# Fytex/Shafa-CD

Measured on AMD Instinct MI355X. Metric: GiB/s Shannon-Fano encode+decode, 64 MiB blocks, 1/2/4/8 GPUs; bit-exact, higher is better.
Workload: dtype u8

## Files before the change

### shafa-cd_amd/csrc/api.hip

```cpp
#include "common.hpp"
#include "internal.hpp"

#include <cmath>
#include <stdio.h>
#include <stdlib.h>

#include <mutex>

static thread_local char g_last_error[512] = "";

int shafa_set_hip_error(hipError_t e, const char *what)
{
    snprintf(g_last_error, sizeof(g_last_error), "%s: %s", what, hipGetErrorString(e));
    return SHAFA_DEVICE_ERROR;
}

int batch_enter(Batch *b, hipStream_t st)
{
    if (!b) return SHAFA_OUTSIDE_MODULE;
    int dev = -1;
    HIP_TRY(hipGetDevice(&dev));
    if (dev != b->device) {
        snprintf(g_last_error, sizeof(g_last_error), "batch of device %d used while device %d is current", b->device, dev);
        return SHAFA_DEVICE_ERROR;
// ... 259 lines not shown

int shafa_hip_set_option(const char *name, long value)
{
    if (name && !strcmp(name, "sf_encode_one_pass_min_blocks")) {
        sfenc_configure(value < 0 ? 0 : (value > (1 << 30) ? (1 << 30) : (int)value));
        return SHAFA_SUCCESS;
    }
    if (name && !strcmp(name, "sf_encode_window_bits")) {
        extern int g_sfe_window_bits;
        if (value < 0 || value > 16) return SHAFA_OUTSIDE_MODULE;
        g_sfe_window_bits = (int)value;
        return SHAFA_SUCCESS;
    }
    if (name && !strcmp(name, "sf_encode_lanes")) {
        if (value != 0 && value != 256 && value != 512) return SHAFA_OUTSIDE_MODULE;
        g_sfe_lanes = (int)value;
        return SHAFA_SUCCESS;
    }
    if (name && !strcmp(name, "sf_decode_path")) {
        if (value < 0 || value > 2) return SHAFA_OUTSIDE_MODULE;
        sfdec_configure_path((int)value);
        return SHAFA_SUCCESS;
    }
    if (name && !strcmp(name, "rle_encode_general")) {
        rleenc_configure(value != 0);
        return SHAFA_SUCCESS;
    }
    if (name && !strcmp(name, "rle_encode_one_pass"))
        return value == 0 ? SHAFA_SUCCESS : SHAFA_OUTSIDE_MODULE;
    if (name && !strcmp(name, "sf_decode_speculate")) {
        sfdec_configure(value <= 0 ? 0 : value >= 2 ? 2 : 1);
        return SHAFA_SUCCESS;
    }
    return SHAFA_OUTSIDE_MODULE;
}

int shafa_hipd_batch_create(int max_blocks, size_t max_block_bytes, shafa_hipd_batch **out)
{
    if (!out || max_blocks <= 0) return SHAFA_OUTSIDE_MODULE;
    Batch *b = (Batch *)calloc(1, sizeof(Batch));
    if (!b) return SHAFA_LACK_OF_MEMORY;
    b->max_blocks = max_blocks;
    b->max_block_bytes = max_block_bytes;
    if (hipGetDevice(&b->device) != hipSuccess) { free(b); return SHAFA_DEVICE_ERROR; }
    b->h_hosterr = (int *)calloc((size_t)max_blocks, sizeof(int));
    if (!b->h_hosterr) { free(b); return SHAFA_LACK_OF_MEMORY; }
    hipError_t e = hipMalloc((void **)&b->d_err, (size_t)max_blocks * sizeof(int));
    if (e == hipSuccess) e = hipMemset(b->d_err, 0, (size_t)max_blocks * sizeof(int));
    if (e == hipSuccess) e = hipMalloc(&b->d_par_hist, (size_t)max_blocks * 48);
    if (e == hipSuccess) e = hipHostMalloc((void **)&b->h_err, (size_t)max_blocks * sizeof(int), hipHostMallocDefault);
    if (e != hipSuccess) {
        if (b->d_err) hipFree(b->d_err);
        free(b);
        return shafa_set_hip_error(e, "shafa_hipd_batch_create");
    }
    *out = (shafa_hipd_batch *)b;
    return SHAFA_SUCCESS;
}

void shafa_hipd_batch_destroy(shafa_hipd_batch *hb)
{
    Batch *b = (Batch *)hb;
    if (!b) return;
    DeviceGuard dg(b->device);
    if (b->has_last) (void)hipStreamSynchronize(b->last_st);
    hipDeviceSynchronize();
// ... 895 lines not shown
```

### shafa-cd_amd/csrc/internal.hpp

```cpp
#pragma once

#include "common.hpp"

#include <string.h>
#include <vector>

struct StageSeg {
    size_t off, bytes;
    hipStream_t st;
    hipEvent_t ev;
    bool sealed;
};

constexpr size_t PARAMS_INLINE_BYTES = 64 * 1024;

struct Batch {
    int device;
    hipStream_t last_st;
    bool has_last;
    int max_blocks;
    size_t max_block_bytes;
    void *d_ws;
    size_t ws_bytes;
    u8 *h_stage;
// ... 200 lines not shown
enum ErrSrc { ERR_PAIR = 0, ERR_QUANT = 1, ERR_ROUND = 2 };
struct ErrorArgs {
    ErrSrc src;
    const u32 *h_mant, *h_keep;
    const double *h_step, *h_bound, *h_abs, *h_rel;
    const u8 *d_ref;
    const u64 *h_ref_off;
};
int planes_error_launch_dev(Batch *bt, hipStream_t st, int nblocks, u32 elem, const ErrorArgs &e, const u8 *d_el, const u64 *h_off,
                            const u64 *h_cap, const u64 *d_n, u64 *d_stat);
int records_launch_dev(Batch *bt, hipStream_t st, int nblocks, u32 width, bool merge, u8 *d_rec, const u64 *h_off, const u64 *h_cap,
                       const u64 *d_n, u8 *d_planes, const u64 *h_plane_off);
int seek_index_launch_dev(Batch *bt, hipStream_t st, int nblocks, const u8 *d_in, const u64 *h_in_off, const u64 *h_in_cap,
                          const u64 *d_in_n, const shafa_code_table *d_tables, u32 span, int flags, const u64 *h_ckpt_first,
                          u64 *d_ckpt, u32 *d_status, u64 *d_out_n);
int read_spans_launch_dev(Batch *bt, hipStream_t st, int nblocks, const u8 *d_file, const u64 *h_pay_off, const u64 *h_pay_n,
                          const u64 *h_n_symbols, const u64 *h_ckpt_first, const shafa_code_table *d_tables, u32 span, int flags,
                          const u64 *d_ckpt, int nitems, const int *h_item_block, const u64 *h_item_first,
                          const u64 *h_item_last, const u64 *h_item_lo, const u64 *h_item_hi, const u64 *h_item_dst, u8 *d_out);
int sfesize_launch_dev(Batch *bt, hipStream_t st, int nblocks, const u64 *d_freq, const shafa_code_table *d_tables, u64 *d_out_n);
struct MoveDesc {
    const u8 *src;
    u8 *dst;
    u64 n;
    u64 hdr_val;
    u32 hdr_len;
    u32 pad;
};
int pack_move_launch(hipStream_t st, int nblocks, const MoveDesc *d_bulk, const MoveDesc *d_seam, const u32 *d_verdict,
                     u64 max_n);
void sfenc_configure(int sfe4_min_blocks);
void sfdec_configure(int speculate);
void sfdec_configure_path(int path);
void rleenc_configure(int force_general);
int gen_launch(hipStream_t st, u64 seed, u64 first, const u8 *d_map, u8 *d_out, size_t n);

int api_lazy_init();
int api_pipe_device(int slot, int n_slots);
```

### shafa-cd_amd/csrc/sf_decode.hip

```cpp
#include <type_traits>
#include "common.hpp"
#include "internal.hpp"

#include <atomic>
#include <mutex>
#include <thread>

#include <algorithm>

#include <stdlib.h>

#include "sfd_common.hpp"
#include "sfd_dp.hpp"
#include "sfd_generic.hpp"

namespace {

typedef __attribute__((address_space(3))) u32 lds_u32;
typedef __attribute__((address_space(3))) u16 lds_u16;
typedef __attribute__((address_space(3))) u8 lds_u8;
template <int LONG> constexpr u32 spec_emask() { return LONG == 2 ? 31u : 15u; }

constexpr int SC_PHW = 16;
constexpr int SC_M = 4;
constexpr int SC_SB = SC_PHW * 4 * SC_M;
constexpr int SC_CH = SC_SB / CH_BYTES;
constexpr int SC_STRIPS_TILE = DTILE / SC_SB;
constexpr int SC_WTILES = 64 / SC_STRIPS_TILE;
constexpr int SC_TILES = DEC_THREADS / SC_STRIPS_TILE;
constexpr int SC_ROWW = SC_PHW + 1;
constexpr int SC_COLB = DEC_THREADS * 4;
constexpr int SC_LDS_ROWS = SC_ROWW * SC_COLB;
constexpr int SC_MISC = 64;
static_assert(SC_COLB == 1024 && SC_WTILES == 2 && SC_STRIPS_TILE == 32, "sfd_scan's lane maps");

struct ScanWin {
    u32 lo, hi, wa, cb;
    __device__ __forceinline__ void init(u32 col) { cb = col; wa = 0xFFFFFFFFu; hi = lo = 0; }
    __device__ __forceinline__ void flush() { wa = 0xFFFFFFFFu; }
    __device__ __forceinline__ u32 at(u32 q)
    {
        const u32 a = cb + ((q >> 5) << 10);
        if (a != wa) {
            lo = *(const lds_u32 *)(size_t)a;
            hi = *(const lds_u32 *)(size_t)(a + SC_COLB);
            wa = a;
        }
        return __builtin_amdgcn_alignbit(hi, lo, q);
    }
};

template <int LONG>
__device__ __forceinline__ u32 scan_long_len(const u16 *lt, ScanWin &sw, const u32 qq)
{
    const u32 win = __builtin_bitreverse32(sw.at(qq));
    const u32 l = (LONG == 1 ? long_code(lt, win) : long_code32(lt, win)) >> 8;
    return l ? l : 1u;
}

template <int LONG>
__device__ __forceinline__ void scan_multi(const lds_u8 *tab, const u16 *lt, const u32 KW, u32 &q, const u32 qe, u32 &cnt, ScanWin &sw)
{
    const u32 q0 = q;
    u32 acc = 0;
    auto multi = [&](auto nlook) {
        constexpr u32 N = decltype(nlook)::value;
        const u32 in_row = 32u * SC_PHW - 1u - (LONG ? (N - 1u) * KW : 0u);
// ... 9 lines not shown
            acc += sum;
            q += sum & 31u;
            if (LONG && __builtin_expect((e & 31u) == 0u, 0)) {
                const u32 l = scan_long_len<LONG>(lt, sw, q);
                q += l;
                acc += l + 32u;
            }
        }
    };
    if (KW <= 10) multi(std::integral_constant<u32, 3>{});
    else multi(std::integral_constant<u32, 2>{});
    cnt += (acc - (q - q0)) >> 5;
}

template <bool LAST, int LONG>
__device__ __forceinline__ bool scan_single(const lds_u8 *tab, const u16 *lt, const u32 KW, u32 &q, const u32 qe, const int qlimit,
                                            u32 &cnt, ScanWin &sw)
{
    const u32 mask = (1u << KW) - 1u;
    const lds_u8 *len0 = tab + (1u << KW);
    while (q < qe) {
        u32 l0 = len0[sw.at(q) & mask];
        if (LONG && __builtin_expect(l0 == 0u, 0)) l0 = scan_long_len<LONG>(lt, sw, q);
        if (LAST && (int)(q + l0) > qlimit) return true;
        q += l0;
        ++cnt;
    }
    return false;
}

#define SC_QUAD 0
#define SC_WAVES 6
#define SC_NT 0
struct ScanIO {
    const u8 *in;
    u64 in_n;
    long long grp_off;
    u32 wbase, ph, cb;
    static constexpr u32 G = SC_QUAD ? 4u : 2u, SPL = 64u / G;
    __device__ __forceinline__ void init(const DecBlk &blk, const u64 wave_off)
    {
        const u32 tid = threadIdx.x, lane = tid & 63u, px = lane / G;
        in = blk.in;
        in_n = blk.in_n;
        ph = lane % G;
        grp_off = (long long)wave_off + (long long)px * SC_SB + 16ll * ph;
        wbase = 4u * ((tid & ~63u) + px);
        cb = 4u * tid;
    }
    template <bool CHECKED>
    __device__ __forceinline__ uint4 fetch16(const long long off) const
    {
        if (!CHECKED || (off >= 0 && (u64)off + 16 <= in_n)) return SC_NT ? gload_nt<uint4>(in + off) : gload<uint4>(in + off);
        u32 w0 = 0, w1 = 0, w2 = 0, w3 = 0;
        if (off >= 0 && (u64)off < in_n) {
            const int nv = (int)(in_n - (u64)off);
#pragma clang loop unroll(disable)
            for (int b = 0; b < nv; ++b) {
                const u32 v = (u32)gload<u8>(in + off + b) << (8 * (b & 3));
                const int wi = b >> 2;
                w0 |= wi == 0 ? v : 0u;
                w1 |= wi == 1 ? v : 0u;
                w2 |= wi == 2 ? v : 0u;
                w3 |= wi == 3 ? v : 0u;
            }
        }
        return make_uint4(w0, w1, w2, w3);
    }
    static __device__ __forceinline__ constexpr u32 sgrp(const int t) { return SC_QUAD ? (u32)t : (u32)t >> 1; }
    static __device__ __forceinline__ constexpr u32 piece(const int t) { return SC_QUAD ? 0u : 32u * ((u32)t & 1u); }
    template <bool CHECKED>
    __device__ __forceinline__ void load_phase(const int k, uint4 (&R)[4]) const
    {
#pragma unroll
        for (int t = 0; t < 4; ++t)
            R[t] = fetch16<CHECKED>(grp_off + (long long)sgrp(t) * SPL * SC_SB + 64ll * k + piece(t));
    }
    template <bool CHECKED>
    __device__ __forceinline__ void load_line(const int j, uint4 (&R)[8]) const
    {
#pragma unroll
        for (int g = 0; g < 2; ++g)
#pragma unroll
            for (int h = 0; h < 2; ++h)
#pragma unroll
                for (int u = 0; u < 2; ++u) {
                    const int t = 2 * g + u;
                    R[4 * h + t] = fetch16<CHECKED>(grp_off + (long long)sgrp(t) * SPL * SC_SB + 64ll * (2 * j + h) + piece(t));
                }
    }
    static constexpr int NRU = SC_QUAD ? 4 : 2;
    template <bool CHECKED>
    __device__ __forceinline__ void load_runup(uint4 (&RU)[NRU]) const
    {
#pragma unroll
        for (int t = 0; t < NRU; ++t) {
            const long long o = grp_off - 32ll - (SC_QUAD ? 16ll * (ph & 2u) : 0ll) + (long long)t * SPL * SC_SB;
            RU[t] = fetch16<CHECKED>(o < 0 ? o + 32 : o);
        }
    }
    __device__ __forceinline__ void put(const u32 r, const u32 xhi, const u32 v) const
    {
        *(lds_u32 *)(size_t)(wbase + r * SC_COLB + 4u * SPL * xhi) = rev_bytes(v);
    }
    __device__ __forceinline__ void wave_sync() const
    {
        __builtin_amdgcn_fence(__ATOMIC_ACQ_REL, "wavefront", "local");
        __builtin_amdgcn_wave_barrier();
    }
    __device__ __forceinline__ void put_runup(const uint4 (&RU)[NRU]) const
    {
#pragma unroll
        for (int t = 0; t < NRU; ++t) {
            const u32 r = 9u + 4u * (ph & 1u);
            if (!SC_QUAD || ph < 2u) {
                put(r, t, RU[t].x);
                put(r + 1, t, RU[t].y);
                put(r + 2, t, RU[t].z);
                put(r + 3, t, RU[t].w);
            }
        }
        wave_sync();
    }
    __device__ __forceinline__ void put_phase(const uint4 *R) const
    {
        const u32 carry = *(const lds_u32 *)(size_t)(cb + 16u * SC_COLB);
        wave_sync();
#pragma unroll
        for (int t = 0; t < 4; ++t) {
            const u32 r = 1u + 4u * ph + piece(t) / 4u;
            put(r, sgrp(t), R[t].x);
            put(r + 1, sgrp(t), R[t].y);
            put(r + 2, sgrp(t), R[t].z);
            put(r + 3, sgrp(t), R[t].w);
        }
        *(lds_u32 *)(size_t)cb = carry;
        wave_sync();
    }
    __device__ __forceinline__ u32 next_strip_word(const uint4 *R, const u64 wave_off) const
    {
        const u32 lane = threadIdx.x & 63u;
        if (ph == 0) {
            if (lane) *(lds_u32 *)(size_t)(wbase - 4u) = rev_bytes(R[0].x);
            *(lds_u32 *)(size_t)(wbase - 4u + 4u * SPL) = rev_bytes(R[2].x);
        }
        wave_sync();
        u32 nw = *(const lds_u32 *)(size_t)cb;
        if (lane == 63) nw = rev_bytes(gload<u32>(in + wave_off + (u64)64 * SC_SB));
        wave_sync();
        return nw;
    }
    __device__ __forceinline__ void put_next_word(const u32 nw_rev) const
    {
        const u32 carry = *(const lds_u32 *)(size_t)(cb + 16u * SC_COLB);
        *(lds_u32 *)(size_t)cb = carry;
        *(lds_u32 *)(size_t)(cb + SC_COLB) = nw_rev;
    }
    template <bool CHECKED>
    __device__ __forceinline__ void put_next_strip(const u64 wave_off) const
    {
        u32 nw = 0;
        const long long off = (long long)wave_off + (long long)((threadIdx.x & 63u) + 1u) * SC_SB;
        if (!CHECKED || (u64)off + 4 <= in_n) nw = gload<u32>(in + off);
        else {
#pragma unroll
            for (int b = 0; b < 4; ++b)
                if ((u64)off + b < in_n) nw |= (u32)gload<u8>(in + off + b) << (8 * b);
        }
        const u32 carry = *(const lds_u32 *)(size_t)(cb + 16u * SC_COLB);
        *(lds_u32 *)(size_t)cb = carry;
        *(lds_u32 *)(size_t)(cb + SC_COLB) = rev_bytes(nw);
    }
};

struct ScanOut {
    u32 e[2], c[4];
    __device__ __forceinline__ void clear() { e[0] = e[1] = 0; c[0] = c[1] = c[2] = c[3] = 0; }
    template <int J> __device__ __forceinline__ void put_ent(const u32 v) { e[J >> 2] |= v << (8 * (J & 3)); }
    template <int J> __device__ __forceinline__ void put_cnt(const u32 v) { c[J >> 1] |= v << (16 * (J & 1)); }
    __device__ __forceinline__ u32 ent(const u32 j) const { return ((j < 4 ? e[0] : e[1]) >> (8u * (j & 3u))) & 0xFFu; }
    __device__ __forceinline__ void set_ent(const u32 j, const u32 v)
    {
        const u32 sh = 8u * (j & 3u), m = ~(0xFFu << sh), x = v << sh;
        if (j < 4) e[0] = (e[0] & m) | x; else e[1] = (e[1] & m) | x;
    }
    __device__ __forceinline__ void set_cnt(const u32 j, const u32 v)
    {
        const u32 sh = 16u * (j & 1u), m = ~(0xFFFFu << sh), x = v << sh, i = j >> 1;
        c[0] = i == 0 ? (c[0] & m) | x : c[0];
        c[1] = i == 1 ? (c[1] & m) | x : c[1];
        c[2] = i == 2 ? (c[2] & m) | x : c[2];
        c[3] = i == 3 ? (c[3] & m) | x : c[3];
    }
    __device__ __forceinline__ u32 total() const
    {
        u32 t = 0;
#pragma unroll
        for (int i = 0; i < 4; ++i) t += (c[i] & 0xFFFFu) + (c[i] >> 16);
        return t;
    }
};
static_assert(SC_CH == 8, "ScanOut packs eight chunks");

template <int LONG>
__device__ __forceinline__ void scan_strip_fast(const lds_u8 *tab, const u16 *lt, const u32 KW, const DecBlk &blk, const u64 wave_off,
                                                const u32 e_forced, const bool forced, ScanOut &o, u32 &exit_)
{
    o.clear();
    ScanIO io;
    io.init(blk, wave_off);
    ScanWin sw;
    sw.init(io.cb);
#ifndef SC_LINE
#define SC_LINE 1
#endif
    uint4 R[SC_LINE ? 8 : 4];
    u32 q, pc = 0;
    auto to_row_end = [&]() {
        scan_multi<LONG>(tab, lt, KW, q, 32u * SC_PHW + 32u, pc, sw);
        if (LONG) scan_single<false, LONG>(tab, lt, KW, q, 32u * SC_PHW, 0, pc, sw);
    };
    {
        uint4 RU[ScanIO::NRU];
        io.load_runup<false>(RU);
#if SC_LINE
        io.load_line<false>(0, R);
#else
        io.load_phase<false>(0, R);
#endif
        io.put_runup(RU);
    }
    static_assert(!SC_QUAD, "next_strip_word: pair mapping");
    const u32 nextw = io.next_strip_word(R, wave_off);
    q = 32u * 9u;
    to_row_end();
    q -= 32u * SC_PHW;
    auto phase = [&](auto kc) {
        constexpr int k = decltype(kc)::value;
#if SC_LINE
        io.put_phase(R + 4 * (k & 1));
        sw.flush();
        if ((k & 1) && k + 1 < SC_M) io.load_line<false>((k + 1) / 2, R);
#else
        io.put_phase(R);
        sw.flush();
        if (k + 1 < SC_M) io.load_phase<false>(k + 1, R);
#endif
        scan_single<false, LONG>(tab, lt, KW, q, 32u, 0, pc, sw);
        if (k > 0) o.put_cnt<(k > 0 ? 2 * k - 1 : 0)>(pc);
        if (k == 0 && forced) q = 32u + e_forced;
        o.put_ent<2 * k>(q - 32u);
        u32 c = 0;
        scan_multi<LONG>(tab, lt, KW, q, 288u, c, sw);
        scan_single<false, LONG>(tab, lt, KW, q, 288u, 0, c, sw);
        o.put_cnt<2 * k>(c);
        o.put_ent<2 * k + 1>(q - 288u);
        pc = 0;
        to_row_end();
        q -= 32u * SC_PHW;
    };
    phase(std::integral_constant<int, 0>{});
    phase(std::integral_constant<int, 1>{});
    phase(std::integral_constant<int, 2>{});
    phase(std::integral_constant<int, 3>{});
    static_assert(SC_M == 4, "four phases written out");
    io.put_next_word(nextw);
    sw.flush();
    scan_single<false, LONG>(tab, lt, KW, q, 32u, 0, pc, sw);
    o.put_cnt<SC_CH - 1>(pc);
    exit_ = (q - 32u) & spec_emask<LONG>();
}

template <int LONG>
__device__ __forceinline__ void scan_strip_redo(const lds_u8 *tab, const u16 *lt, const u32 KW, const DecBlk &blk, const u64 wave_off,
                                                const u32 e_forced, bool walking, ScanOut &o, u32 &exit_)
{
    ScanIO io;
    io.init(blk, wave_off);
    ScanWin sw;
    sw.init(io.cb);
    uint4 R[4];
    u32 q = 0, pc = 0;
#pragma clang loop unroll(disable)
    for (int k = 0; k < SC_M; ++k) {
        io.load_phase<false>(k, R);
        io.put_phase(R);
        sw.flush();
        if (walking) {
            if (k == 0) {
                q = 32u + e_forced;
                o.set_ent(0, e_forced);
            } else {
                scan_single<false, LONG>(tab, lt, KW, q, 32u, 0, pc, sw);
                o.set_cnt(2 * k - 1, pc);
                const u32 e = q - 32u;
                if (e == o.ent(2 * k)) walking = false; else o.set_ent(2 * k, e);
            }
        }
        if (walking) {
            u32 c = 0;
            scan_multi<LONG>(tab, lt, KW, q, 288u, c, sw);
            scan_single<false, LONG>(tab, lt, KW, q, 288u, 0, c, sw);
            o.set_cnt(2 * k, c);
            const u32 e = q - 288u;
            if (e == o.ent(2 * k + 1)) walking = false; else o.set_ent(2 * k + 1, e);
        }
        if (walking) {
            pc = 0;
            scan_multi<LONG>(tab, lt, KW, q, 32u * SC_PHW + 32u, pc, sw);
            if (LONG) scan_single<false, LONG>(tab, lt, KW, q, 32u * SC_PHW, 0, pc, sw);
            q -= 32u * SC_PHW;
        }
        if (!__any(walking)) return;
    }
    io.put_next_strip<false>(wave_off);
    sw.flush();
    if (walking) {
        scan_single<false, LONG>(tab, lt, KW, q, 32u, 0, pc, sw);
        o.set_cnt(SC_CH - 1, pc);
        exit_ = (q - 32u) & spec_emask<LONG>();
    }
}

template <int LONG>
__device__ __forceinline__ void scan_unit(u8 *smem, const DecBlk &blk, const u32 wtile, u8 *__restrict__ chunk_entry,
                                          u16 *__restrict__ chunk_cnt, u32 *__restrict__ tile_cnt, u8 *__restrict__ tile_guess,
                                          u8 *__restrict__ tile_exit, const u32 tab_bytes)
{
    const u32 lane = threadIdx.x & 63u;
    const size_t gtw = (size_t)blk.tile_base + wtile;
    const u32 KW = blk.KW;
    const lds_u8 *tab = (const lds_u8 *)(size_t)SC_LDS_ROWS;
    const u16 *lt = (const u16 *)(smem + SC_LDS_ROWS + tab_bytes + SC_MISC);
    const u64 wave_off = (u64)wtile * DTILE;
    const u64 left = blk.in_n > wave_off ? blk.in_n - wave_off : 0;
    if (left < (u64)64 * SC_SB + 4) return;
    const bool forced = wtile == 0 && lane == 0;
    ScanOut o;
    u32 exit_ = 0;
    scan_strip_fast<LONG>(tab, lt, KW, blk, wave_off, 0u, forced, o, exit_);
    bool bad = false;
    for (int round = 0; round < 3; ++round) {
        const u32 prev = (u32)__shfl_up((int)exit_, 1, 64);
        bad = lane > 0 && (o.e[0] & 0xFFu) != prev;
        if (!__any(bad) || round == 2) break;
        scan_strip_redo<LONG>(tab, lt, KW, blk, wave_off, prev, bad, o, exit_);
    }
    if (__any(bad)) {
        if (lane == 0) __hip_atomic_store(blk.run_dp, 1u, __ATOMIC_RELAXED, __HIP_MEMORY_SCOPE_AGENT);
    }
    const u32 my_tile = wtile + lane / SC_STRIPS_TILE;
    const u32 incl = dpp_scan_add(o.total());
    const u32 half = (u32)__builtin_amdgcn_readlane((int)incl, 31);
    if (my_tile < blk.n_tiles) {
        const size_t c0 = gtw * DEC_THREADS + (size_t)lane * SC_CH;
        gstore<uint2>(chunk_entry + c0, make_uint2(o.e[0], o.e[1]));
        gstore<uint4>(chunk_cnt + c0, make_uint4(o.c[0], o.c[1], o.c[2], o.c[3]));
    }
    const bool two = wtile + 1 < blk.n_tiles;
    if (lane == 0) tile_guess[gtw] = (u8)(o.e[0] & 0xFFu);
    if (lane == 31) {
        tile_cnt[gtw] = half;
        if (two) { tile_exit[gtw] = 0; tile_guess[gtw + 1] = 0; }
    }
    if (lane == 63) {
        if (two) tile_cnt[gtw + 1] = incl - half;
        tile_exit[gtw + (two ? 1 : 0)] = (u8)exit_;
    }
}

template <int LONG>
__global__ __launch_bounds__(DEC_THREADS) __attribute__((amdgpu_waves_per_eu(SC_WAVES, 8))) void sfd_scan(const DecBlk *__restrict__ blks, u8 *__restrict__ chunk_entry,
                                                        u16 *__restrict__ chunk_cnt, u32 *__restrict__ tile_cnt,
                                                        u8 *__restrict__ tile_guess, u8 *__restrict__ tile_exit, u32 tab_bytes, u32 long_bytes)
{
    extern __shared__ __attribute__((aligned(16))) u8 smem[];
    const DecBlk blk = blks[blockIdx.y];
    if (!blk.run_dp || __hip_atomic_load(blk.run_dp, __ATOMIC_RELAXED, __HIP_MEMORY_SCOPE_AGENT) != 0) return;
    if (lds_addr(smem) != 0) __builtin_trap();
    const u32 wv = threadIdx.x >> 6;
    const u32 t_lo = blockIdx.x * SC_TILES;
    if (t_lo >= blk.n_tiles) return;
    fill_lds16((void *)(smem + SC_LDS_ROWS), (const void *)blk.cnt3, 2u << blk.KW);
    if (LONG) {
        u16 *lt = (u16 *)(smem + SC_LDS_ROWS + tab_bytes + SC_MISC);
        const u16 *src = LONG == 1 ? blk.longtab : blk.long32;
        if (src) fill_lds16((void *)lt, src, long_bytes);
        else if (threadIdx.x == 0) *lt = 0;
    }
    lds_barrier();
    const u32 wtile = t_lo + wv * SC_WTILES;
    if (wtile < blk.n_tiles) scan_unit<LONG>(smem, blk, wtile, chunk_entry, chunk_cnt, tile_cnt, tile_guess, tile_exit, tab_bytes);
}

constexpr int SL_SW = 16;
constexpr int SL_ROW = SL_SW + 1;
constexpr int SL_STRIPS = DEC_THREADS + 1;
constexpr int SL_LDS_DATA = (SL_STRIPS * SL_ROW + 3) / 4 * 16;
constexpr int SL_MISC = DEC_THREADS + 16 + 32;

struct SlWin {
    u32 lo, hi, wa;
    __device__ __forceinline__ void init() { wa = 0xFFFFFFFFu; hi = lo = 0; }
    __device__ __forceinline__ u32 at(u32 q)
    {
        const u32 a = (q >> 3) & ~3u;
        if (a != wa) {
            const lds_u32 *pa = (const lds_u32 *)(size_t)a;
            lo = pa[0];
            hi = pa[1];
            wa = a;
        }
        return __builtin_amdgcn_alignbit(hi, lo, q);
    }
};

template <int LONG>
__device__ __forceinline__ void sl_walk(const lds_u8 *tab, const u16 *lt, const u32 KW, u32 &q, const u32 qe, const int qlimit, u32 &cnt, SlWin &sw)
{
    const u32 mask = (1u << KW) - 1u;
    auto long_len = [&](const u32 qq) -> u32 {
        const u32 win = __builtin_bitreverse32(sw.at(qq));
        const u32 l = (LONG == 1 ? long_code(lt, win) : long_code32(lt, win)) >> 8;
        return l ? l : 1u;
    };
// ... 732 lines not shown
    }
    u64 rs = key | 1ull;
    int fails = 0;
    for (int trial = 0; trial < SPEC_TRIALS && fails <= SPEC_MAX_FAILS; ++trial) {
        u64 w[SPEC_WORDS];
        for (u64 &x : w) x = spec_rand(rs);
        if (!spec_trial(w, h.lenlut.data(), h.K1)) ++fails;
    }
    const bool yes = fails <= SPEC_MAX_FAILS;
    std::lock_guard<std::mutex> lk(cmu);
    ckey[slot] = key;
    cval[slot] = yes ? 2 : 1;
    return yes;
}

struct SfdArrays {
    u8 *cfn, *tfn;
    u8 *tent, *cent;
    u16 *ccnt;
    u32 *tcnt;
    u64 *toff;
    u8 *tguess, *texit;
};

enum SfdForm { SFD_MID32, SFD_LONG_ALL, SFD_PACKED12, SFD_PACKED13, SFD_PACKED };

static u32 sfd_tpw(u32 most, u32 max_tiles, int nblocks)
{
    u32 tpw = most;
    while (tpw > 1 && (u64)ceil_div_u64(max_tiles, tpw) * nblocks < 2048) tpw >>= 1;
    return tpw;
}

static void sfd_launch_packed(hipStream_t st, const DecBlk *dblk, int nblocks, u32 max_tiles, SfdForm form, bool esc, bool spec,
                              u32 tabb, u32 long_used, bool all_spec, u32 ws_tab, u32 ws_cap, const SfdArrays &a, bool one = false)
{
    static decltype(&sfd_scan<0>) const scans[3] = {sfd_scan<2>, sfd_scan<1>, sfd_scan<0>};
    static decltype(&sfd_ends<0>) const ends[3] = {sfd_ends<2>, sfd_ends<1>, sfd_ends<0>};
    static decltype(&sfd_sync16<true, false>) const syncs[4] = {sfd_sync16<false, true>, sfd_sync16<true, false, 12>,
                                                                sfd_sync16<true, false, 13>, sfd_sync16<true, false>};
    const int f = form < SFD_PACKED12 ? form : 2;
    const dim3 grid_b((u32)nblocks), wg(DEC_THREADS);
    hipLaunchKernelGGL(sfd_tables, dim3((u32)nblocks, 8), wg, 0, st, dblk);
    if (spec) {
        const size_t lds_scan = (size_t)SC_LDS_ROWS + tabb + SC_MISC + long_used;
        const size_t lds_ends = (size_t)SL_LDS_DATA + tabb + SL_MISC + long_used;
        hipLaunchKernelGGL(scans[f], dim3((u32)ceil_div_u64(max_tiles, SC_TILES), (u32)nblocks), wg, lds_scan, st, dblk, a.cent, a.ccnt,
                           a.tcnt, a.tguess, a.texit, tabb, long_used);
        hipLaunchKernelGGL(ends[f], dim3(1u + (u32)ceil_div_u64(max_tiles, SF_LINKS), (u32)nblocks), wg, lds_ends, st, dblk, a.cent,
                           a.ccnt, a.tcnt, a.tguess, a.texit, tabb, long_used);
    }
    const u32 tpw = all_spec ? 256u : sfd_tpw(4, max_tiles, nblocks);
    const dim3 grid_f((u32)ceil_div_u64(max_tiles, tpw), (u32)nblocks);
    if (form == SFD_MID32) {
        hipLaunchKernelGGL(sfd_sync32, grid_f, wg, 0, st, dblk, a.cfn, a.tfn, tpw);
        hipLaunchKernelGGL(sfd_tiles, grid_b, wg, (size_t)32 * DEC_THREADS + DEC_THREADS, st, dblk, 32u, (const u8 *)a.tfn, a.tent);
        hipLaunchKernelGGL(sfd_countfsm32, grid_f, wg, 0, st, dblk, (const u8 *)a.cfn, (const u8 *)a.tent, a.cent, a.ccnt, a.tcnt, tpw);
    } else {
        constexpr int CSUBS = 4;
        hipLaunchKernelGGL(syncs[form - SFD_LONG_ALL], grid_f, wg, 0, st, dblk, (u64 *)a.cfn, (u64 *)a.tfn, tpw);
        hipLaunchKernelGGL(sfd_tiles16, grid_b, wg, 0, st, dblk, (const u64 *)a.tfn, a.tent);
        hipLaunchKernelGGL((sfd_countfsm<CSUBS>), dim3((u32)ceil_div_u64(max_tiles, tpw * CSUBS), (u32)nblocks), dim3(DEC_THREADS * CSUBS),
                           0, st, dblk, (const u64 *)a.cfn, (const u8 *)a.tent, a.cent, a.ccnt, a.tcnt, tpw);
    }
    hipLaunchKernelGGL(sfd_offsets, grid_b, wg, 0, st, dblk, (const u32 *)a.tcnt, a.toff);
    static decltype(&sfd_wstage<0, false>) const wstages[5] = {sfd_wstage<2, true>, sfd_wstage<1, true>, sfd_wstage<0, true>,
                                                               sfd_wstage<0, false>, sfd_wstage<0, false, true>};
    const u32 tpw_ws = sfd_tpw(16, max_tiles, nblocks);
    const size_t lds_ws = (size_t)ws_rows_bytes(esc) + ws_tab + ws_cap + WS_MISC + long_used;
    hipLaunchKernelGGL(wstages[one ? 4 : f == 2 && !esc ? 3 : f], dim3((u32)ceil_div_u64(max_tiles, tpw_ws), (u32)nblocks), wg, lds_ws, st,
                       dblk, (const u8 *)a.cent, (const u16 *)a.ccnt, (const u64 *)a.toff, tpw_ws, ws_tab, ws_cap, long_used);
}

static int sfd_launch_bytemap(hipStream_t st, const DecBlk *dblk, u32 nb, u32 max_tiles, u32 R, u32 l2cap, const SfdArrays &a)
{
    const size_t lds_lut = (size_t)(1u << LUT_MAXK) * 2 + (size_t)l2cap * 2;
    const size_t lds_sync = (size_t)LDS_DATA + (size_t)R * DEC_THREADS + lds_lut + 4 * R + 64;
    const size_t lds_count = lds_sync + DEC_THREADS;
    const size_t lds_write = (size_t)LDS_DATA + lds_lut + 64;
    const size_t lds_tiles = (size_t)R * DEC_THREADS + DEC_THREADS;
    if (lds_tiles > 65536 || lds_sync > 65536) {
// ... 214 lines not shown
        if (spec_blk[b] && hblk_kw[b] > k1_max) k1_max = hblk_kw[b];
        k1_all = (k1_all == 0 || k1_all == tabs[b].K1) ? tabs[b].K1 : 0xFFFFFFFFu;
        if (!spec_blk[b]) all_spec = false;
    }
    const SfdForm form = mid32 ? SFD_MID32 : long_all ? SFD_LONG_ALL : k1_all == 12 ? SFD_PACKED12 : k1_all == 13 ? SFD_PACKED13
                                                                                                          : SFD_PACKED;
    u32 ws_tab = 16;
    for (int b = 0; b < nblocks; ++b) {
        const u32 k3 = sym3_window(tabs[b].K1), tb = (ws_one ? 2u : 4u) << k3;
        if (tb > ws_tab) ws_tab = tb;
    }
    u32 ws_cap = 4096, ws_tight = 4096;
    for (int b = 0; b < nblocks; ++b) {
        if (!ntiles[b]) continue;
        const u64 per_tile = ceil_div_u64(h_n_symbols[b], ntiles[b]);
        const u64 c = per_tile + per_tile / 8 + 1024, t = per_tile + per_tile / 32 + 256;
        if (c > ws_cap) ws_cap = (u32)(c > 40960 ? 40960 : c);
        if (t > ws_tight) ws_tight = (u32)(t > 40960 ? 40960 : t);
    }
    {
        const u32 base = (u32)ws_rows_bytes(ws_esc) + ws_tab + long_used + (u32)WS_MISC;
        const u32 most = 65536u - base;
        if (ws_cap > most) ws_cap = most;
        constexpr u32 steps[3] = {20480u, 26880u, 40960u};
        for (u32 k = 0; k < 3; ++k) {
            if (base + ((ws_tight + 15u) & ~15u) <= steps[k]) {
                ws_cap = steps[k] - base;
                if (ws_cap > most) ws_cap = most;
                break;
            }
        }
    }
    ws_cap &= ~15u;
    sfd_launch_packed(st, dblk, nblocks, max_tiles, form, ws_esc, any_spec, 2u << k1_max, long_used, all_spec, ws_tab, ws_cap, arr, ws_one);
    HIP_TRY(hipGetLastError());
    return pscope.done();
}

#include "sfd_dev.hpp"
```

Baseline: 896.4.

## Let each scan lane walk multiple consecutive strips to cut speculation seams

```diff
diff --git a/shafa-cd_amd/csrc/api.hip b/shafa-cd_amd/csrc/api.hip
--- a/shafa-cd_amd/csrc/api.hip
+++ b/shafa-cd_amd/csrc/api.hip
@@ -315,6 +315,11 @@
         sfdec_configure(value <= 0 ? 0 : value >= 2 ? 2 : 1);
         return SHAFA_SUCCESS;
     }
+    if (name && !strcmp(name, "sf_scan_strips")) {
+        if (value != 0 && value != 1 && value != 2 && value != 4) return SHAFA_OUTSIDE_MODULE;
+        sfdec_configure_scan_strips((int)value);
+        return SHAFA_SUCCESS;
+    }
     return SHAFA_OUTSIDE_MODULE;
 }
 
diff --git a/shafa-cd_amd/csrc/internal.hpp b/shafa-cd_amd/csrc/internal.hpp
--- a/shafa-cd_amd/csrc/internal.hpp
+++ b/shafa-cd_amd/csrc/internal.hpp
@@ -256,6 +256,7 @@
 void sfenc_configure(int sfe4_min_blocks);
 void sfdec_configure(int speculate);
 void sfdec_configure_path(int path);
+void sfdec_configure_scan_strips(int strips);
 void rleenc_configure(int force_general);
 int gen_launch(hipStream_t st, u64 seed, u64 first, const u8 *d_map, u8 *d_out, size_t n);
 
diff --git a/shafa-cd_amd/csrc/sf_decode.hip b/shafa-cd_amd/csrc/sf_decode.hip
--- a/shafa-cd_amd/csrc/sf_decode.hip
+++ b/shafa-cd_amd/csrc/sf_decode.hip
@@ -33,6 +33,9 @@
 constexpr int SC_LDS_ROWS = SC_ROWW * SC_COLB;
 constexpr int SC_MISC = 64;
 static_assert(SC_COLB == 1024 && SC_WTILES == 2 && SC_STRIPS_TILE == 32, "sfd_scan's lane maps");
+constexpr int SC_SMAX = 4;
+template <int S> constexpr bool sc_strips_ok() { return S >= 1 && S <= SC_SMAX && SC_STRIPS_TILE % S == 0 && 64 % (SC_STRIPS_TILE / S) == 0; }
+static_assert(sc_strips_ok<1>() && sc_strips_ok<2>() && sc_strips_ok<4>(), "a lane's sub-strips lie in one tile, a unit is whole tiles");
 
 struct ScanWin {
     u32 lo, hi, wa, cb;
@@ -108,19 +111,27 @@
 #define SC_QUAD 0
 #define SC_WAVES 6
 #define SC_NT 0
+__device__ __forceinline__ u32 sc_tid_again()
+{
+    u32 t = threadIdx.x;
+    asm volatile("" : "+v"(t));
+    return t;
+}
+template <int S>
 struct ScanIO {
+    static constexpr long long SB = (long long)S * SC_SB;
     const u8 *in;
     u64 in_n;
     long long grp_off;
     u32 wbase, ph, cb;
     static constexpr u32 G = SC_QUAD ? 4u : 2u, SPL = 64u / G;
-    __device__ __forceinline__ void init(const DecBlk &blk, const u64 wave_off)
-    {
-        const u32 tid = threadIdx.x, lane = tid & 63u, px = lane / G;
+    __device__ __forceinline__ void init(const DecBlk &blk, const u64 wave_off, const u32 tid = threadIdx.x)
+    {
+        const u32 lane = tid & 63u, px = lane / G;
         in = blk.in;
         in_n = blk.in_n;
         ph = lane % G;
-        grp_off = (long long)wave_off + (long long)px * SC_SB + 16ll * ph;
+        grp_off = (long long)wave_off + (long long)px * SB + 16ll * ph;
         wbase = 4u * ((tid & ~63u) + px);
         cb = 4u * tid;
     }
@@ -150,7 +161,7 @@
     {
 #pragma unroll
         for (int t = 0; t < 4; ++t)
-            R[t] = fetch16<CHECKED>(grp_off + (long long)sgrp(t) * SPL * SC_SB + 64ll * k + piece(t));
+            R[t] = fetch16<CHECKED>(grp_off + (long long)sgrp(t) * SPL * SB + 64ll * k + piece(t));
     }
     template <bool CHECKED>
     __device__ __forceinline__ void load_line(const int j, uint4 (&R)[8]) const
@@ -162,7 +173,7 @@
 #pragma unroll
                 for (int u = 0; u < 2; ++u) {
                     const int t = 2 * g + u;
-                    R[4 * h + t] = fetch16<CHECKED>(grp_off + (long long)sgrp(t) * SPL * SC_SB + 64ll * (2 * j + h) + piece(t));
+                    R[4 * h + t] = fetch16<CHECKED>(grp_off + (long long)sgrp(t) * SPL * SB + 64ll * (2 * j + h) + piece(t));
                 }
     }
     static constexpr int NRU = SC_QUAD ? 4 : 2;
@@ -171,7 +182,7 @@
     {
 #pragma unroll
         for (int t = 0; t < NRU; ++t) {
-            const long long o = grp_off - 32ll - (SC_QUAD ? 16ll * (ph & 2u) : 0ll) + (long long)t * SPL * SC_SB;
+            const long long o = grp_off - 32ll - (SC_QUAD ? 16ll * (ph & 2u) : 0ll) + (long long)t * SPL * SB;
             RU[t] = fetch16<CHECKED>(o < 0 ? o + 32 : o);
         }
     }
@@ -222,7 +233,7 @@
         }
         wave_sync();
         u32 nw = *(const lds_u32 *)(size_t)cb;
-        if (lane == 63) nw = rev_bytes(gload<u32>(in + wave_off + (u64)64 * SC_SB));
+        if (lane == 63) nw = rev_bytes(gload<u32>(in + wave_off + (u64)64 * SB));
         wave_sync();
         return nw;
     }
@@ -236,7 +247,7 @@
     __device__ __forceinline__ void put_next_strip(const u64 wave_off) const
     {
         u32 nw = 0;
-        const long long off = (long long)wave_off + (long long)((threadIdx.x & 63u) + 1u) * SC_SB;
+        const long long off = (long long)wave_off + (long long)((threadIdx.x & 63u) + 1u) * SB;
         if (!CHECKED || (u64)off + 4 <= in_n) nw = gload<u32>(in + off);
         else {
 #pragma unroll
@@ -254,11 +265,12 @@
     __device__ __forceinline__ void clear() { e[0] = e[1] = 0; c[0] = c[1] = c[2] = c[3] = 0; }
     template <int J> __device__ __forceinline__ void put_ent(const u32 v) { e[J >> 2] |= v << (8 * (J & 3)); }
     template <int J> __device__ __forceinline__ void put_cnt(const u32 v) { c[J >> 1] |= v << (16 * (J & 1)); }
-    __device__ __forceinline__ u32 ent(const u32 j) const { return ((j < 4 ? e[0] : e[1]) >> (8u * (j & 3u))) & 0xFFu; }
+    __device__ __forceinline__ u32 ent(const u32 j) const { return (u32)((((u64)e[1] << 32) | e[0]) >> (8u * j)) & 0xFFu; }
     __device__ __forceinline__ void set_ent(const u32 j, const u32 v)
     {
-        const u32 sh = 8u * (j & 3u), m = ~(0xFFu << sh), x = v << sh;
-        if (j < 4) e[0] = (e[0] & m) | x; else e[1] = (e[1] & m) | x;
+        const u64 all = (((u64)e[1] << 32) | e[0]) & ~((u64)0xFFu << (8u * j)), x = (u64)v << (8u * j);
+        e[0] = (u32)(all | x);
+        e[1] = (u32)((all | x) >> 32);
     }
     __device__ __forceinline__ void set_cnt(const u32 j, const u32 v)
     {
@@ -275,15 +287,34 @@
         for (int i = 0; i < 4; ++i) t += (c[i] & 0xFFFFu) + (c[i] >> 16);
         return t;
     }
+    __device__ __forceinline__ void store(u8 *__restrict__ chunk_entry, u16 *__restrict__ chunk_cnt, const size_t c0) const
+    {
+        gstore<uint2>(chunk_entry + c0, make_uint2(e[0], e[1]));
+        gstore<uint4>(chunk_cnt + c0, make_uint4(c[0], c[1], c[2], c[3]));
+    }
+    __device__ __forceinline__ void load(const u8 *chunk_entry, const u16 *chunk_cnt, const size_t c0)
+    {
+        const uint2 a = gload<uint2>(chunk_entry + c0);
+        const uint4 b = gload<uint4>(chunk_cnt + c0);
+        e[0] = a.x; e[1] = a.y;
+        c[0] = b.x; c[1] = b.y; c[2] = b.z; c[3] = b.w;
+    }
+};
+struct ScanLane {
+    u8 *chunk_entry;
+    u16 *chunk_cnt;
+    u32 cot;
+    __device__ __forceinline__ u32 co() const { return cot & 0xFFFFu; }
+    __device__ __forceinline__ u32 tot() const { return cot >> 16; }
 };
 static_assert(SC_CH == 8, "ScanOut packs eight chunks");
 
-template <int LONG>
+template <int LONG, int S>
 __device__ __forceinline__ void scan_strip_fast(const lds_u8 *tab, const u16 *lt, const u32 KW, const DecBlk &blk, const u64 wave_off,
-                                                const u32 e_forced, const bool forced, ScanOut &o, u32 &exit_)
+                                                const u32 e_forced, const bool forced, ScanOut &o, u32 &exit_, ScanLane &ln)
 {
     o.clear();
-    ScanIO io;
+    ScanIO<S> io;
     io.init(blk, wave_off);
     ScanWin sw;
     sw.init(io.cb);
@@ -297,12 +328,12 @@
         if (LONG) scan_single<false, LONG>(tab, lt, KW, q, 32u * SC_PHW, 0, pc, sw);
     };
     {
-        uint4 RU[ScanIO::NRU];
-        io.load_runup<false>(RU);
+        uint4 RU[ScanIO<S>::NRU];
+        io.template load_runup<false>(RU);
 #if SC_LINE
-        io.load_line<false>(0, R);
+        io.template load_line<false>(0, R);
 #else
-        io.load_phase<false>(0, R);
+        io.template load_phase<false>(0, R);
 #endif
         io.put_runup(RU);
     }
@@ -311,20 +342,26 @@
     q = 32u * 9u;
     to_row_end();
     q -= 32u * SC_PHW;
-    auto phase = [&](auto kc) {
+    auto phase = [&](auto kc, const int s) {
         constexpr int k = decltype(kc)::value;
 #if SC_LINE
         io.put_phase(R + 4 * (k & 1));
         sw.flush();
-        if ((k & 1) && k + 1 < SC_M) io.load_line<false>((k + 1) / 2, R);
+        if ((k & 1) && (k + 1 < SC_M || s + 1 < S)) io.template load_line<false>((k + 1) / 2, R);
 #else
         io.put_phase(R);
         sw.flush();
-        if (k + 1 < SC_M) io.load_phase<false>(k + 1, R);
+        if (k + 1 < SC_M || s + 1 < S) io.template load_phase<false>(k + 1, R);
 #endif
         scan_single<false, LONG>(tab, lt, KW, q, 32u, 0, pc, sw);
         if (k > 0) o.put_cnt<(k > 0 ? 2 * k - 1 : 0)>(pc);
-        if (k == 0 && forced) q = 32u + e_forced;
+        if (S > 1 && k == 0 && s > 0) {
+            o.put_cnt<SC_CH - 1>(pc);
+            o.store(ln.chunk_entry, ln.chunk_cnt, ln.co() - SC_CH);
+            ln.cot += o.total() << 16;
+            o.clear();
+        }
+        if (k == 0 && s == 0 && forced) q = 32u + e_forced;
         o.put_ent<2 * k>(q - 32u);
         u32 c = 0;
         scan_multi<LONG>(tab, lt, KW, q, 288u, c, sw);
@@ -335,51 +372,98 @@
         to_row_end();
         q -= 32u * SC_PHW;
     };
-    phase(std::integral_constant<int, 0>{});
-    phase(std::integral_constant<int, 1>{});
-    phase(std::integral_constant<int, 2>{});
-    phase(std::integral_constant<int, 3>{});
+    if constexpr (S == 1) {
+        phase(std::integral_constant<int, 0>{}, 0);
+        phase(std::integral_constant<int, 1>{}, 0);
+        phase(std::integral_constant<int, 2>{}, 0);
+        phase(std::integral_constant<int, 3>{}, 0);
+    } else {
+        auto sub_strip = [&](const int s) {
+            phase(std::integral_constant<int, 0>{}, s);
+            phase(std::integral_constant<int, 1>{}, s);
+            phase(std::integral_constant<int, 2>{}, s);
+            phase(std::integral_constant<int, 3>{}, s);
+            io.grp_off += SC_SB;
+            ln.cot += SC_CH;
+            asm volatile("" : "+v"(io.grp_off), "+v"(ln.cot));
+        };
+        sub_strip(0);
+        sub_strip(1);
+        if constexpr (S == 4) {
+            sub_strip(2);
+            sub_strip(3);
+        }
+        static_assert(S == 1 || S == 2 || S == 4, "the sub-strips written out");
+    }
     static_assert(SC_M == 4, "four phases written out");
     io.put_next_word(nextw);
     sw.flush();
     scan_single<false, LONG>(tab, lt, KW, q, 32u, 0, pc, sw);
     o.put_cnt<SC_CH - 1>(pc);
     exit_ = (q - 32u) & spec_emask<LONG>();
-}
-
-template <int LONG>
+    if (S > 1) {
+        o.store(ln.chunk_entry, ln.chunk_cnt, ln.co() - SC_CH);
+        ln.cot += o.total() << 16;
+    }
+}
+
+template <int LONG, int S>
 __device__ __forceinline__ void scan_strip_redo(const lds_u8 *tab, const u16 *lt, const u32 KW, const DecBlk &blk, const u64 wave_off,
-                                                const u32 e_forced, bool walking, ScanOut &o, u32 &exit_)
-{
-    ScanIO io;
-    io.init(blk, wave_off);
+                                                const u32 e_forced, bool walking, ScanOut &w, u32 &exit_, ScanLane &ln)
+{
+    const u32 tid = S == 1 ? threadIdx.x : sc_tid_again();
+    ScanIO<S> io;
+    io.init(blk, wave_off, tid);
     ScanWin sw;
     sw.init(io.cb);
     uint4 R[4];
     u32 q = 0, pc = 0;
+    const u32 co = (tid & 63u) * (S * SC_CH);
+    if (S > 1) w.load(ln.chunk_entry, ln.chunk_cnt, co);
+    u32 w_tot = S > 1 ? w.total() : 0u;
+    bool dirty = walking, to_end = true;
+    int s = 0;
 #pragma clang loop unroll(disable)
-    for (int k = 0; k < SC_M; ++k) {
-        io.load_phase<false>(k, R);
+    for (int kk = 0; kk < S * SC_M; ++kk) {
+        const int k = kk & (SC_M - 1);
+        io.template load_phase<false>(kk, R);
         io.put_phase(R);
         sw.flush();
-        if (walking) {
-            if (k == 0) {
+        if (S > 1 && k == 0 && kk > 0) {
+            if (walking) {
+                scan_single<false, LONG>(tab, lt, KW, q, 32u, 0, pc, sw);
+                w.set_cnt(SC_CH - 1, pc);
+            }
+            if (dirty) {
+                w.store(ln.chunk_entry, ln.chunk_cnt, co + (u32)s * SC_CH);
+                ln.cot += (w.total() - w_tot) << 16;
+            }
+            ++s;
+            w.load(ln.chunk_entry, ln.chunk_cnt, co + (u32)s * SC_CH);
+            w_tot = w.total();
+            dirty = walking;
+            if (walking) {
+                const u32 e = q - 32u;
+                if (e == w.ent(0)) walking = false; else w.set_ent(0, e);
+            }
+        } else if (walking) {
+            if (kk == 0) {
                 q = 32u + e_forced;
-                o.set_ent(0, e_forced);
+                w.set_ent(0, e_forced);
             } else {
                 scan_single<false, LONG>(tab, lt, KW, q, 32u, 0, pc, sw);
-                o.set_cnt(2 * k - 1, pc);
+                w.set_cnt(2 * k - 1, pc);
                 const u32 e = q - 32u;
-                if (e == o.ent(2 * k)) walking = false; else o.set_ent(2 * k, e);
+                if (e == w.ent(2 * k)) walking = false; else w.set_ent(2 * k, e);
             }
         }
         if (walking) {
             u32 c = 0;
             scan_multi<LONG>(tab, lt, KW, q, 288u, c, sw);
             scan_single<false, LONG>(tab, lt, KW, q, 288u, 0, c, sw);
-            o.set_cnt(2 * k, c);
+            w.set_cnt(2 * k, c);
             const u32 e = q - 288u;
-            if (e == o.ent(2 * k + 1)) walking = false; else o.set_ent(2 * k + 1, e);
+            if (e == w.ent(2 * k + 1)) walking = false; else w.set_ent(2 * k + 1, e);
         }
         if (walking) {
             pc = 0;
@@ -387,18 +471,41 @@
             if (LONG) scan_single<false, LONG>(tab, lt, KW, q, 32u * SC_PHW, 0, pc, sw);
             q -= 32u * SC_PHW;
         }
-        if (!__any(walking)) return;
-    }
-    io.put_next_strip<false>(wave_off);
-    sw.flush();
-    if (walking) {
-        scan_single<false, LONG>(tab, lt, KW, q, 32u, 0, pc, sw);
-        o.set_cnt(SC_CH - 1, pc);
-        exit_ = (q - 32u) & spec_emask<LONG>();
-    }
-}
-
-template <int LONG>
+        if (!__any(walking)) { to_end = false; break; }
+    }
+    if (to_end) {
+        io.template put_next_strip<false>(wave_off);
+        sw.flush();
+        if (walking) {
+            scan_single<false, LONG>(tab, lt, KW, q, 32u, 0, pc, sw);
+            w.set_cnt(SC_CH - 1, pc);
+            exit_ = (q - 32u) & spec_emask<LONG>();
+        }
+    }
+    if (S > 1 && dirty) {
+        w.store(ln.chunk_entry, ln.chunk_cnt, co + (u32)s * SC_CH);
+        ln.cot += (w.total() - w_tot) << 16;
+    }
+}
+
+template <int SEG>
+__device__ __forceinline__ u32 dpp_seg_sum(u32 v)
+{
+    static_assert(SEG == 8 || SEG == 16, "a run of lanes inside one DPP row");
+    v += (u32)__builtin_amdgcn_update_dpp(0, (int)v, 0x111, 0xf, 0xf, false);
+    v += (u32)__builtin_amdgcn_update_dpp(0, (int)v, 0x112, 0xf, 0xf, false);
+    v += (u32)__builtin_amdgcn_update_dpp(0, (int)v, 0x114, 0xf, 0xf, false);
+    if (SEG == 16) v += (u32)__builtin_amdgcn_update_dpp(0, (int)v, 0x118, 0xf, 0xf, false);
+    return v;
+}
+
+template <int S>
+__device__ __forceinline__ u32 scan_tiles_of(const u64 in_n)
+{
+    return in_n < 4 ? 0u : (u32)((in_n - 4) / ((u64)64 * S * SC_SB)) * (u32)(SC_WTILES * S);
+}
+
+template <int LONG, int S>
 __device__ __forceinline__ void scan_unit(u8 *smem, const DecBlk &blk, const u32 wtile, u8 *__restrict__ chunk_entry,
                                           u16 *__restrict__ chunk_cnt, u32 *__restrict__ tile_cnt, u8 *__restrict__ tile_guess,
                                           u8 *__restrict__ tile_exit, const u32 tab_bytes)
@@ -410,53 +517,66 @@
     const u16 *lt = (const u16 *)(smem + SC_LDS_ROWS + tab_bytes + SC_MISC);
     const u64 wave_off = (u64)wtile * DTILE;
     const u64 left = blk.in_n > wave_off ? blk.in_n - wave_off : 0;
-    if (left < (u64)64 * SC_SB + 4) return;
+    if (left < (u64)64 * S * SC_SB + 4) return;
     const bool forced = wtile == 0 && lane == 0;
     ScanOut o;
+    ScanLane ln = {chunk_entry + gtw * DEC_THREADS, chunk_cnt + gtw * DEC_THREADS, lane * (S * SC_CH)};
     u32 exit_ = 0;
-    scan_strip_fast<LONG>(tab, lt, KW, blk, wave_off, 0u, forced, o, exit_);
+    scan_strip_fast<LONG, S>(tab, lt, KW, blk, wave_off, 0u, forced, o, exit_, ln);
     bool bad = false;
+    u32 guess = 0;
     for (int round = 0; round < 3; ++round) {
         const u32 prev = (u32)__shfl_up((int)exit_, 1, 64);
-        bad = lane > 0 && (o.e[0] & 0xFFu) != prev;
+        if (S > 1) guess = gload<u8>(ln.chunk_entry + lane * (S * SC_CH));
+        bad = lane > 0 && (S == 1 ? o.e[0] & 0xFFu : guess) != prev;
         if (!__any(bad) || round == 2) break;
-        scan_strip_redo<LONG>(tab, lt, KW, blk, wave_off, prev, bad, o, exit_);
+        scan_strip_redo<LONG, S>(tab, lt, KW, blk, wave_off, prev, bad, o, exit_, ln);
     }
     if (__any(bad)) {
         if (lane == 0) __hip_atomic_store(blk.run_dp, 1u, __ATOMIC_RELAXED, __HIP_MEMORY_SCOPE_AGENT);
     }
-    const u32 my_tile = wtile + lane / SC_STRIPS_TILE;
-    const u32 incl = dpp_scan_add(o.total());
-    const u32 half = (u32)__builtin_amdgcn_readlane((int)incl, 31);
-    if (my_tile < blk.n_tiles) {
-        const size_t c0 = gtw * DEC_THREADS + (size_t)lane * SC_CH;
-        gstore<uint2>(chunk_entry + c0, make_uint2(o.e[0], o.e[1]));
-        gstore<uint4>(chunk_cnt + c0, make_uint4(o.c[0], o.c[1], o.c[2], o.c[3]));
-    }
-    const bool two = wtile + 1 < blk.n_tiles;
-    if (lane == 0) tile_guess[gtw] = (u8)(o.e[0] & 0xFFu);
-    if (lane == 31) {
-        tile_cnt[gtw] = half;
-        if (two) { tile_exit[gtw] = 0; tile_guess[gtw + 1] = 0; }
-    }
-    if (lane == 63) {
-        if (two) tile_cnt[gtw + 1] = incl - half;
-        tile_exit[gtw + (two ? 1 : 0)] = (u8)exit_;
-    }
-}
-
-template <int LONG>
+    if constexpr (S == 1) {
+        const u32 my_tile = wtile + lane / SC_STRIPS_TILE;
+        const u32 incl = dpp_scan_add(o.total());
+        const u32 half = (u32)__builtin_amdgcn_readlane((int)incl, 31);
+        if (my_tile < blk.n_tiles) o.store(ln.chunk_entry, ln.chunk_cnt, ln.co());
+        const bool two = wtile + 1 < blk.n_tiles;
+        if (lane == 0) tile_guess[gtw] = (u8)(o.e[0] & 0xFFu);
+        if (lane == 31) {
+            tile_cnt[gtw] = half;
+            if (two) { tile_exit[gtw] = 0; tile_guess[gtw + 1] = 0; }
+        }
+        if (lane == 63) {
+            if (two) tile_cnt[gtw + 1] = incl - half;
+            tile_exit[gtw + (two ? 1 : 0)] = (u8)exit_;
+        }
+    } else {
+        constexpr u32 SEG = SC_STRIPS_TILE / S, NT = SC_WTILES * S;
+        const u32 tsum = dpp_seg_sum<(int)SEG>(ln.tot());
+        const u32 l = sc_tid_again() & 63u, t = l / SEG;
+        if (l % SEG == 0) tile_guess[gtw + t] = t == 0 ? (u8)guess : (u8)0;
+        if (l % SEG == SEG - 1) {
+            tile_cnt[gtw + t] = tsum;
+            tile_exit[gtw + t] = t == NT - 1 ? (u8)exit_ : (u8)0;
+        }
+    }
+}
+
+template <int LONG, int S = 1>
 __global__ __launch_bounds__(DEC_THREADS) __attribute__((amdgpu_waves_per_eu(SC_WAVES, 8))) void sfd_scan(const DecBlk *__restrict__ blks, u8 *__restrict__ chunk_entry,
                                                         u16 *__restrict__ chunk_cnt, u32 *__restrict__ tile_cnt,
-                                                        u8 *__restrict__ tile_guess, u8 *__restrict__ tile_exit, u32 tab_bytes, u32 long_bytes)
+                                                        u8 *__restrict__ tile_guess, u8 *__restrict__ tile_exit, u32 tab_bytes, u32 long_bytes,
+                                                        u32 tail_wgs)
 {
     extern __shared__ __attribute__((aligned(16))) u8 smem[];
     const DecBlk blk = blks[blockIdx.y];
     if (!blk.run_dp || __hip_atomic_load(blk.run_dp, __ATOMIC_RELAXED, __HIP_MEMORY_SCOPE_AGENT) != 0) return;
     if (lds_addr(smem) != 0) __builtin_trap();
-    const u32 wv = threadIdx.x >> 6;
-    const u32 t_lo = blockIdx.x * SC_TILES;
-    if (t_lo >= blk.n_tiles) return;
+    const u32 wv = S == 1 ? threadIdx.x >> 6 : (u32)__builtin_amdgcn_readfirstlane((int)(threadIdx.x >> 6));
+    const bool tail = S > 1 && blockIdx.x < tail_wgs;
+    const u32 t_lo = S == 1 ? blockIdx.x * SC_TILES
+                            : tail ? scan_tiles_of<S>(blk.in_n) + blockIdx.x * SC_TILES : (blockIdx.x - tail_wgs) * (SC_TILES * S);
+    if (t_lo >= (S == 1 || tail ? blk.n_tiles : scan_tiles_of<S>(blk.in_n))) return;
     fill_lds16((void *)(smem + SC_LDS_ROWS), (const void *)blk.cnt3, 2u << blk.KW);
     if (LONG) {
         u16 *lt = (u16 *)(smem + SC_LDS_ROWS + tab_bytes + SC_MISC);
@@ -465,8 +585,13 @@
         else if (threadIdx.x == 0) *lt = 0;
     }
     lds_barrier();
-    const u32 wtile = t_lo + wv * SC_WTILES;
-    if (wtile < blk.n_tiles) scan_unit<LONG>(smem, blk, wtile, chunk_entry, chunk_cnt, tile_cnt, tile_guess, tile_exit, tab_bytes);
+    if (S > 1 && tail) {
+        const u32 wtile = t_lo + wv * SC_WTILES;
+        if (wtile < blk.n_tiles) scan_unit<LONG, 1>(smem, blk, wtile, chunk_entry, chunk_cnt, tile_cnt, tile_guess, tile_exit, tab_bytes);
+        return;
+    }
+    const u32 wtile = t_lo + wv * (SC_WTILES * S);
+    if (wtile < blk.n_tiles) scan_unit<LONG, S>(smem, blk, wtile, chunk_entry, chunk_cnt, tile_cnt, tile_guess, tile_exit, tab_bytes);
 }
 
 constexpr int SL_SW = 16;
@@ -1265,10 +1390,62 @@
     return tpw;
 }
 
+typedef decltype(&sfd_scan<0>) SfdScanFn;
+static u32 sfd_scan_strips_max(int) { return 2u; }
+static SfdScanFn sfd_scan_kernel(int f, u32 strips)
+{
+    static SfdScanFn const scans[2][3] = {{sfd_scan<2>, sfd_scan<1>, sfd_scan<0>}, {sfd_scan<2, 2>, sfd_scan<1, 2>, sfd_scan<0, 2>}};
+    return scans[strips == 2 ? 1 : 0][f];
+}
+
+static int g_sfd_scan_strips = 0;
+void sfdec_configure_scan_strips(int strips) { g_sfd_scan_strips = strips; }
+static u32 sfd_scan_strips(int device, int f, size_t lds_scan, int nblocks, const u64 *h_in_n, const std::vector<char> &spec_blk)
+{
+    if (g_sfd_scan_strips) return std::min((u32)g_sfd_scan_strips, sfd_scan_strips_max(f));
+    constexpr u64 ROUNDS = 8;
+    auto units = [&](u32 S) {
+        u64 n = 0;
+        for (int b = 0; b < nblocks; ++b)
+            if (spec_blk[b] && h_in_n[b] >= 4) n += (h_in_n[b] - 4) / ((u64)64 * S * SC_SB);
+        return n;
+    };
+    constexpr int MAXDEV = 64;
+    if (device < 0 || device >= MAXDEV) return 1;
+    static std::mutex mu;
+    static int cus_by_dev[MAXDEV];
+    static std::vector<std::pair<u64, int>> occ_cache;
+    for (u32 S = sfd_scan_strips_max(f); S > 1; S >>= 1) {
+        const u64 n = units(S);
+        if (n < ROUNDS * 64) continue;
+        int occ = 0, cus = 0;
+        {
+            std::lock_guard<std::mutex> lk(mu);
+            if (!cus_by_dev[device]) {
+                hipDeviceProp_t prop;
+                if (hipGetDeviceProperties(&prop, device) != hipSuccess) return 1;
+                cus_by_dev[device] = prop.multiProcessorCount;
+            }
+            cus = cus_by_dev[device];
+            const u64 key = ((u64)device << 56) | ((u64)f << 52) | ((u64)S << 48) | (u64)lds_scan;
+            for (const auto &c : occ_cache)
+                if (c.first == key) occ = c.second;
+            if (!occ) {
+                if (hipOccupancyMaxActiveBlocksPerMultiprocessor(&occ, (const void *)sfd_scan_kernel(f, S), DEC_THREADS, lds_scan) != hipSuccess ||
+                    occ < 1)
+                    return 1;
+                occ_cache.emplace_back(key, occ);
+            }
+        }
+        if (n >= ROUNDS * (u64)cus * (u64)occ * (DEC_THREADS / 64)) return S;
+    }
+    return 1;
+}
+
 static void sfd_launch_packed(hipStream_t st, const DecBlk *dblk, int nblocks, u32 max_tiles, SfdForm form, bool esc, bool spec,
-                              u32 tabb, u32 long_used, bool all_spec, u32 ws_tab, u32 ws_cap, const SfdArrays &a, bool one = false)
-{
-    static decltype(&sfd_scan<0>) const scans[3] = {sfd_scan<2>, sfd_scan<1>, sfd_scan<0>};
+                              u32 tabb, u32 long_used, bool all_spec, u32 ws_tab, u32 ws_cap, const SfdArrays &a, bool one = false,
+                              u32 strips = 1)
+{
     static decltype(&sfd_ends<0>) const ends[3] = {sfd_ends<2>, sfd_ends<1>, sfd_ends<0>};
     static decltype(&sfd_sync16<true, false>) const syncs[4] = {sfd_sync16<false, true>, sfd_sync16<true, false, 12>,
                                                                 sfd_sync16<true, false, 13>, sfd_sync16<true, false>};
@@ -1278,8 +1455,13 @@
     if (spec) {
         const size_t lds_scan = (size_t)SC_LDS_ROWS + tabb + SC_MISC + long_used;
         const size_t lds_ends = (size_t)SL_LDS_DATA + tabb + SL_MISC + long_used;
-        hipLaunchKernelGGL(scans[f], dim3((u32)ceil_div_u64(max_tiles, SC_TILES), (u32)nblocks), wg, lds_scan, st, dblk, a.cent, a.ccnt,
-                           a.tcnt, a.tguess, a.texit, tabb, long_used);
+        if (strips > 1) {
+            const u32 tail_wgs = (u32)ceil_div_u64(SC_WTILES * strips + 1, SC_TILES);
+            hipLaunchKernelGGL(sfd_scan_kernel(f, strips), dim3(tail_wgs + (u32)ceil_div_u64(max_tiles, SC_TILES * strips), (u32)nblocks), wg,
+                               lds_scan, st, dblk, a.cent, a.ccnt, a.tcnt, a.tguess, a.texit, tabb, long_used, tail_wgs);
+        } else
+            hipLaunchKernelGGL(sfd_scan_kernel(f, 1), dim3((u32)ceil_div_u64(max_tiles, SC_TILES), (u32)nblocks), wg, lds_scan, st, dblk, a.cent, a.ccnt,
+                               a.tcnt, a.tguess, a.texit, tabb, long_used, 0u);
         hipLaunchKernelGGL(ends[f], dim3(1u + (u32)ceil_div_u64(max_tiles, SF_LINKS), (u32)nblocks), wg, lds_ends, st, dblk, a.cent,
                            a.ccnt, a.tcnt, a.tguess, a.texit, tabb, long_used);
     }
@@ -1560,7 +1742,12 @@
         }
     }
     ws_cap &= ~15u;
-    sfd_launch_packed(st, dblk, nblocks, max_tiles, form, ws_esc, any_spec, 2u << k1_max, long_used, all_spec, ws_tab, ws_cap, arr, ws_one);
+    u32 strips = 1;
+    if (any_spec)
+        strips = sfd_scan_strips(bt->device, form < SFD_PACKED12 ? form : 2, (size_t)SC_LDS_ROWS + (2u << k1_max) + SC_MISC + long_used,
+                                 nblocks, h_in_n, spec_blk);
+    sfd_launch_packed(st, dblk, nblocks, max_tiles, form, ws_esc, any_spec, 2u << k1_max, long_used, all_spec, ws_tab, ws_cap, arr, ws_one,
+                      strips);
     HIP_TRY(hipGetLastError());
     return pscope.done();
 }
```

After: 904.0, median of 6. About the same (+0.8%).
